# GTEC-UDC/roskfpos

Hardware: AMD Instinct MI355X
Metric: EKF predict+update steps/s at 65536 tags x 8 anchors; RMS pos err vs CPU ref (higher is better)
Workload: dtype f64 arithmetic; f64 state and covariance, f32/int32 measurements in HBM (KFPOS_STORE_MIXED)

## Files before the change

### __graft_entry__.py

```python
from __future__ import annotations

import os
import shutil
import subprocess
import sys

ROOT = os.path.dirname(os.path.abspath(__file__))
CSRC = os.path.join(ROOT, "roskfpos_amd", "csrc")
HIP_LIB = os.path.join(CSRC, "libkfpos_hip.so")
ADAPTOR_DEMO = os.path.join(CSRC, "kfpos_replay")


def _stale(target, sources):
    if not os.path.exists(target):
        return True
    mt = os.path.getmtime(target)
    return any(os.path.getmtime(s) > mt for s in sources if os.path.exists(s))


def build(force: bool = False) -> None:
    jobs = str(min(8, os.cpu_count() or 1))
    res = subprocess.run(["make", "-s", "-j", jobs, "-C", CSRC] + (["-B"] if force else []) + ["all"],
                         capture_output=True, text=True)
    if res.returncode != 0:
        sys.stderr.write(res.stdout + res.stderr)
        raise subprocess.CalledProcessError(res.returncode, res.args)
    res = subprocess.run(["make", "-s", "-C", CSRC, "check"], capture_output=True, text=True)
    if res.returncode != 0:
        sys.stderr.write(res.stdout + res.stderr)
        if os.path.exists(HIP_LIB):
            os.remove(HIP_LIB)
        raise RuntimeError("a build-time performance rule is broken (scratch inside a loop / a kernel lost its second "
                           "wavefront per SIMD): " + (res.stdout + res.stderr).strip())
    subprocess.check_call(["make", "-s", "-C", os.path.join(ROOT, "oracle")] + (["-B"] if force else []))
    import glob
    core_headers = sorted(glob.glob(os.path.join(CSRC, "kfpos_core*.h"))) + [os.path.join(CSRC, "kfpos_p48.h")]
    emu_dir = os.path.join(ROOT, "tests", "emu")
    emu_so = os.path.join(emu_dir, "libkfpos_emu.so")
    if force or _stale(emu_so, [os.path.join(emu_dir, "kfpos_emu.cpp")] + core_headers):
        subprocess.check_call(["g++", "-O2", "-std=c++17", "-fPIC", "-shared", "-Wno-unknown-pragmas",
                               "-o", emu_so, os.path.join(emu_dir, "kfpos_emu.cpp")])
    fake_dir = os.path.join(ROOT, "tests", "fake_rccl")
    fake_so = os.path.join(fake_dir, "libfake_rccl.so")
    if force or _stale(fake_so, [os.path.join(fake_dir, "fake_rccl.cpp")]):
        subprocess.check_call([shutil.which("hipcc") or "/opt/rocm/bin/hipcc", "-O2", "-std=c++17", "-shared", "-fPIC",
                               "-o", fake_so, os.path.join(fake_dir, "fake_rccl.cpp"), "-lrt"])
    if ROOT not in sys.path:
        sys.path.insert(0, ROOT)
    import roskfpos_amd
    from roskfpos_amd import capi
    capi.load()


def smoke() -> None:
    if ROOT not in sys.path:
        sys.path.insert(0, ROOT)
    sys.path.insert(0, os.path.join(ROOT, "oracle"))
    import numpy as np
    from roskfpos_amd import capi
    from roskfpos_amd.synth import Workload
    import oracle_py

    T, A, S = 256, 8, 12
    w = Workload(T, A)
    for model in (capi.MODEL_TOA, capi.MODEL_TOA_IMU):
        bank = capi.KfposBank(model, T, w.anchors, init_pos=w.init_positions())
        orc = oracle_py.OracleBank(model, T, w.anchors, init_pos=w.init_positions(), n_threads=4)
        err, cov = w.err_est(), w.accel_cov()
        for s in range(S):
            r, a, dt = w.ranges_mm(s), w.accel(s), w.dt_of(s)
            if model == capi.MODEL_TOA_IMU:
                bank.step_toa_imu(r, err, a, cov, dt)
                orc.step_imu(a, cov, 0.0)
                orc.step_toa(r, err, dt)
            else:
                bank.step_toa(r, err, dt)
                orc.step_toa(r, err, dt)
        x, _, _ = bank.get_state()
        xo, _ = orc.get_state()
        rms = float(np.sqrt(((x[:, :3] - xo[:, :3]) ** 2).sum(1).mean()))
        print(f"smoke model={model}: RMS position difference vs oracle = {rms:.3e} m")
        assert rms <= 1e-6, rms
        bank.close()


if __name__ == "__main__":
    build()
    if len(sys.argv) > 1 and sys.argv[1] == "smoke":
        smoke()
```

### roskfpos_amd/csrc/kfpos_core_imu9.h

```cpp
#ifndef KFPOS_CORE_IMU9_H
#define KFPOS_CORE_IMU9_H

namespace kfpos {

constexpr double INFO_FORM_MIN_PIVOT = 1e-7;

struct Tag9 {
    double pos[3], vel[3];
    Cov<9, true> P;
};
struct Imu {
    bool has;
    double acc[3];
    double *ci;
    int ci_stride;
    KFPOS_HD double Wi(int k) const { return ci[(6 + k) * ci_stride]; }
};

KFPOS_FN void imu_whitener(const double s[9], double *ci, int ci_stride) {
    double c00, c11, c22, i00, i11, i22;
    kf_sqrt_rsqrt(s[0], c00, i00);
    const double c10 = s[3] * i00, c20 = s[6] * i00;
    kf_sqrt_rsqrt(s[4] - c10 * c10, c11, i11);
    const double c21 = (s[7] - c20 * c10) * i11;
// ... 618 lines not shown
    Iekf9Iter it;
    KFPOS_UNROLL
    for (int k = 0; k < 6; ++k) { it.ve[k] = 0.0; it.wl[k] = 0.0; o.mrlast[k] = 0.0; }
    it.qd = 0.0;
    it.cost = 1e20;
    o.dlast[0] = o.dlast[1] = o.dlast[2] = 0.0;
    o.gain_iters = 0;
#if defined(__HIP_DEVICE_COMPILE__)
    constexpr bool PAIRS = RANGING && SC::NA == 8 && SC::CHUNK == 0 && !SC::COOP;
    const bool pairs = PAIRS && pr.pair_anchor_tab && __builtin_amdgcn_ballot_w64(true) == ~0ull;
#endif
    bool more = true;
    int stop = max_steps;
#if defined(__HIP_DEVICE_COMPILE__)
    if (pairs) stop = 8 < max_steps ? 8 : max_steps;
#endif
    for (;;) {
        while (more && o.gain_iters < stop) {
            Iekf9Parked pk;
            iekf9_fetch<false>(binv, binv_stride, imu, pk);
            const double p[3] = {xhat[0] + it.ve[0], xhat[1] + it.ve[1], xhat[2] + it.ve[2]};
            Sweep9 sw;
            iekf9_sweep<RANGING>(p, sc, pr, sw);
            more = iekf9_pass<DIAG>(xhat, pk, imu, tol, sw, it, o);
        }
#if defined(__HIP_DEVICE_COMPILE__)
        if constexpr (PAIRS) {
            if (pairs) {
                const uint64_t m = __builtin_amdgcn_ballot_w64(more && o.gain_iters < max_steps);
                if (m == 0) break;
                if (__popcll(m) <= 32) {
                    iekf9_pairs<DIAG, ACC0>(m, xhat, binv, binv_stride, sc, pr.pair_anchor_tab, imu, max_steps, tol, it, o);
                    break;
                }
                stop = stop + 4 < max_steps ? stop + 4 : max_steps;
                continue;
            }
        }
#endif
        break;
    }
    KFPOS_UNROLL
    for (int k = 0; k < 6; ++k) o.w[k] = it.wl[k];
    o.cost = it.cost;
}

KFPOS_FN void cov_update9(Cov<9, true> &P, const double mr[6], const double d[3], const Imu &imu) {
    Factor9 f;
    factor9(mr, d, imu, f);
    KFPOS_UNROLL
    for (int k = 0; k < 6; ++k) {
        double pt[9], s = 1.0;
        KFPOS_UNROLL
        for (int i = 0; i < 9; ++i) {
            double v = 0.0;
            KFPOS_UNROLL
            for (int l = 0; l < 6; ++l) {
                const bool nz = (l < 3 && k < 3 && l >= k) || (l >= 3 && k >= 3 && l <= k);
                if (nz) v += P(i, e9(l)) * L9(f, l, k);
            }
            pt[i] = v;
        }
        KFPOS_UNROLL
        for (int l = 0; l < 6; ++l) {
            const bool nz = (l < 3 && k < 3 && l >= k) || (l >= 3 && k >= 3 && l <= k);
            if (nz) s += L9(f, l, k) * pt[e9(l)];
        }
        const double is = kf_rcp(s);
        KFPOS_UNROLL
        for (int i = 0; i < 9; ++i) {
            const double pi = pt[i] * is;
            KFPOS_UNROLL
            for (int j = i; j < 9; ++j) P(i, j) -= pi * pt[j];
        }
    }
}

struct CovPark9 {
    double *a;
    int stride;
};

template <bool RANGING, class SC>
KFPOS_FN uint32_t step_imu9(Tag9 &tg, SC &sc, const Params &pr, double dt, const Imu &imu, const CovPark9 &park) {
    constexpr bool has_ranging = RANGING;
    const int n_valid = has_ranging ? count_used(sc, pr, 0) : 0;
    if (!pr.use_init_pos && (isnan(tg.pos[0]) || isnan(tg.pos[1]))) {
        if (!has_ranging) return 0;
        if (n_valid < 4) return ST_FEW_RANGES;
        double p[3] = {1.0, 1.0, 4.0}, sse, c[6];
        set_weights_ml(sc, pr, 0ull);
        const int it = ml_estimate(p, sc, pr, 0, n_valid, sse);
        if (ml_covariance_throws(sc, pr, 0, n_valid, sse)) return ST_UPDATE_SKIPPED;
        if (!ml_covariance(p, sc, pr, sse, c)) return ST_UPDATE_SKIPPED;
        tg.pos[0] = p[0]; tg.pos[1] = p[1]; tg.pos[2] = p[2];
        tg.P(0, 0) = c[0]; tg.P(0, 1) = c[1]; tg.P(1, 1) = c[3];
        return pack_status(ST_ML_INIT, 0, it, -1);
    }
    const double c = dt * dt / 2;
    double xhat[9];
    KFPOS_UNROLL
    for (int k = 0; k < 3; ++k) {
        xhat[k] = tg.pos[k] + dt * tg.vel[k] + c * 0.0;
        xhat[3 + k] = tg.vel[k] + dt * 0.0;
        xhat[6 + k] = 0.0;
    }
    predict9(tg.P, dt, pr.jolt);
    Cov<6, true> B;
    KFPOS_UNROLL
    for (int i = 0; i < 6; ++i) {
        KFPOS_UNROLL
        for (int j = i; j < 6; ++j) B(i, j) = tg.P(e9(i), e9(j));
    }
    KFPOS_UNROLL
    for (int k = 0; k < 45; ++k) park.a[k * park.stride] = tg.P.a[k];
    double *binv = park.a + 45 * park.stride;
    const bool invertible = sym6_inverse(B, binv, park.stride, INFO_FORM_MIN_PIVOT);
    Iekf9Out o;
    iekf9_weights(xhat, sc, pr, has_ranging, n_valid, o);
    if (o.flags & ST_UPDATE_SKIPPED) {
        KFPOS_UNROLL
        for (int k = 0; k < 45; ++k) tg.P.a[k] = park.a[k * park.stride];
        return ST_UPDATE_SKIPPED;
    }
    if (invertible) {
        iekf9_info<false, RANGING, true>(xhat, binv, park.stride, sc, pr, imu, 20, 1e-4, o);
        KFPOS_UNROLL
        for (int k = 0; k < 45; ++k) tg.P.a[k] = park.a[k * park.stride];
    } else {
        KFPOS_UNROLL
        for (int k = 0; k < 45; ++k) tg.P.a[k] = park.a[k * park.stride];
        iekf9<false, RANGING>(xhat, tg.P, sc, pr, imu, 20, 1e-4, o);
    }
    KFPOS_UNROLL
    for (int i = 0; i < 6; ++i) {
        double v = 0.0;
        KFPOS_UNROLL
        for (int k = 0; k < 6; ++k) v += tg.P(i, e9(k)) * o.w[k];
        if (i < 3) tg.pos[i] = xhat[i] + v;
        else tg.vel[i - 3] = xhat[i] + v;
    }
    cov_update9(tg.P, o.mrlast, o.dlast, imu);
    return pack_status(o.flags, o.gain_iters, o.ml_iters, -1);
}

KFPOS_FN void pose9(const Tag9 &tg, double t, double jolt, double pos[3], double vel[3], double cov[9]) {
    const double c = t * t / 2, t3 = (t * t * t) / 6;
    KFPOS_UNROLL
    for (int i = 0; i < 3; ++i) {
        pos[i] = tg.pos[i] + t * tg.vel[i];
        vel[i] = tg.vel[i];
        KFPOS_UNROLL
        for (int j = 0; j < 3; ++j) {
            const Cov<9, true> &P = tg.P;
            const double xpp = P(i, j) + t * P(3 + i, j) + c * P(6 + i, j);
            const double xpv = P(i, 3 + j) + t * P(3 + i, 3 + j) + c * P(6 + i, 3 + j);
            const double xpa = P(i, 6 + j) + t * P(3 + i, 6 + j) + c * P(6 + i, 6 + j);
            cov[3 * i + j] = xpp + t * xpv + c * xpa + (i == j ? jolt * t3 * t3 : 0.0);
        }
    }
}

}
#endif
```

### roskfpos_amd/csrc/kfpos_hip.hip

```cpp
#include <algorithm>
#include <cmath>
#include <cstdio>
#include <cstdlib>
#include <cstring>
#include <new>
#include <string>
#include <type_traits>
#include <vector>

#include "kfpos_kernels.h"

std::string &kfpos_error_text() {
    thread_local std::string text;
    return text;
}

namespace {

#define g_err (kfpos_error_text())

#define HIPCHK(expr)                                                                              \
    do {                                                                                          \
        hipError_t e_ = (expr);                                                                   \
        if (e_ != hipSuccess) {                                                                   \
            g_err = std::string(#expr) + ": " + hipGetErrorString(e_);                            \
            return KFPOS_ERR_HIP;                                                                 \
        }                                                                                         \
    } while (0)

}


namespace {

size_t lds_bytes(const kfpos_handle *h) { return (size_t)3 * h->cfg.max_anchors * WAVE * sizeof(double); }
size_t park_bytes() { return (size_t)36 * WAVE * sizeof(double); }
size_t park9_bytes() { return (size_t)78 * WAVE * sizeof(double) + 24 * sizeof(double); }

void fill_args(const kfpos_handle *h, KArgs &a) {
    std::memcpy(a.anchors, h->anchors, sizeof(a.anchors));
    a.T = h->cfg.n_tags;
    a.A = h->have_anchors ? h->A : 0;
    a.accel_noise = h->cfg.accel_noise;
    a.jolt = h->cfg.jolt;
    a.cost_threshold = h->cfg.cost_threshold;
    a.ignore_worst = h->cfg.ignore_worst;
    a.top_n = h->cfg.top_n;
    a.ml_variant = h->cfg.model == KFPOS_MODEL_ML ? h->cfg.ml_variant : 0;
    a.pair9 = h->pair9 ? 1 : 0;
    a.use_init_pos = h->cfg.use_init_pos;
    a.use_fixed_height = h->planar.use_fixed_height;
    a.imu_fixed_cov_acc = h->planar.imu_use_fixed_cov_acc;
    a.imu_fixed_cov_w = h->planar.imu_use_fixed_cov_ang_vel_z;
    a.px4_height = h->planar.px4_height;
    a.px4_arm_p1 = h->planar.px4_arm_p1;
    a.px4_arm_p2 = h->planar.px4_arm_p2;
    a.px4_cov_vel = h->planar.px4_cov_velocity;
    a.px4_cov_gyro_z = h->planar.px4_cov_gyro_z;
    a.imu_cov_acc = h->planar.imu_cov_acc;
    a.imu_cov_w = h->planar.imu_cov_ang_vel_z;
    a.mag_offset = h->planar.mag_angle_offset;
    a.mag_cov = h->planar.mag_cov;
    a.platch = h->d_latch;
    a.sensor = nullptr;
    a.pos = h->d_pos;
    a.vel = h->d_vel;
    a.P = h->d_P;
    a.flags = h->d_flags;
    a.imu_acc = h->d_imu_acc;
    a.imu_cov = h->d_imu_cov;
    a.ranges = nullptr;
    a.err = nullptr;
    a.dt = nullptr;
    a.dt_shared = 0.0;
    a.accel = nullptr;
    a.cov = nullptr;
    a.mode = MODE_TOA;
    a.latch = 1;
    a.status = nullptr;
    a.n_steps = 1;
    a.stride_ranges = a.stride_err = a.stride_accel = a.stride_cov = 0;
    a.traj = nullptr;
}


bool toa6_two_waves(const kfpos_handle *h) {
    return h->two_waves && h->cfg.model == KFPOS_MODEL_TOA && !h->full && !h->force_generic && !h->coop &&
           h->cfg.max_anchors == 8 && h->cfg.ignore_worst == 0 && h->cfg.top_n == 0;
}
int static_anchors(const kfpos_handle *h) {
    if (h->cfg.max_anchors == 8) return 8;
    if (h->cfg.max_anchors == 16 && h->cfg.model == KFPOS_MODEL_TOA) return -16;
    return 0;
}

step_kernel_t step_kernel(const kfpos_handle *h, bool sensor_call = false, bool imu_only = false) {
    const int st = h->cfg.storage, as = (h->force_generic || sensor_call) ? 0 : static_anchors(h);
    if (h->cfg.model == KFPOS_MODEL_PLANAR) return kfpos_k::planar_kernel(st, h->planar_sensors || sensor_call, as);
    if (h->cfg.model == KFPOS_MODEL_ML) return kfpos_k::ml_kernel(st, as);
    if (h->coop) return kfpos_k::toa6_coop_kernel(st);
    if (h->cfg.model == KFPOS_MODEL_TOA) {
        const int heur = h->cfg.ignore_worst != 0 ? 2 : (h->cfg.top_n != 0 ? 1 : 0);
        if (h->full) return kfpos_k::toa6_full_kernel(st, as, heur);
        return kfpos_k::toa6_sym_kernel(st, as, heur, toa6_two_waves(h));
    }
    return kfpos_k::imu9_kernel(st, as, !imu_only);
}

int launch_step(kfpos_handle *h, const KArgs &a, hipStream_t s) {
    if (h->coop) {
        const int groups = (a.T + COOP_TAGS_PER_WAVE - 1) / COOP_TAGS_PER_WAVE;
        hipLaunchKernelGGL(step_kernel(h), dim3(groups), dim3(WAVE), 0, s, a);
        HIPCHK(hipGetLastError());
        h->stepped = true;
        return KFPOS_OK;
    }
    const int blocks = (a.T + WAVE - 1) / WAVE;
    const bool generic = h->force_generic || static_anchors(h) <= 0 || (h->cfg.model == KFPOS_MODEL_TOA && h->full) ||
                         (h->cfg.model == KFPOS_MODEL_PLANAR && h->planar_sensors) || toa6_two_waves(h);
    const bool planar_sensor = h->cfg.model == KFPOS_MODEL_PLANAR && a.mode != 0;
    size_t lds = (a.mode == MODE_IMU_ONLY || planar_sensor || !generic) ? 0 : lds_bytes(h);
    if (lds && h->cfg.model == KFPOS_MODEL_TOA && !h->force_generic && static_anchors(h) != 0 && h->msz == 4)
        lds = lds * 5 / 6;
    if (h->cfg.model == KFPOS_MODEL_PLANAR && (h->planar_sensors || planar_sensor)) lds += park_bytes();
    if (h->cfg.model == KFPOS_MODEL_TOA && h->full) lds += park_bytes();
    if (toa6_two_waves(h)) lds += (size_t)(h->msz == 4 ? 19 : 15) * WAVE * sizeof(double);
    if (h->cfg.model == KFPOS_MODEL_TOA_IMU) lds += park9_bytes();
    hipLaunchKernelGGL(step_kernel(h, planar_sensor, a.mode == MODE_IMU_ONLY && h->cfg.model == KFPOS_MODEL_TOA_IMU), dim3(blocks), dim3(WAVE), lds, s, a);
    HIPCHK(hipGetLastError());
    h->stepped = true;
    return KFPOS_OK;
}
// ... 116 lines not shown

inline int pidx(const kfpos_handle *h, int i, int j) {
    if (h->full) return i * h->n + j;
    const int N = h->n;
    if (i > j) { const int tt = i; i = j; j = tt; }
    return i * N - i * (i - 1) / 2 + (j - i);
}

}

extern "C" {

const char *kfpos_last_error(void) { return g_err.c_str(); }
const char *kfpos_strerror(int code) {
    switch (code) {
    case KFPOS_OK: return "ok";
    case KFPOS_ERR_ARG: return "invalid argument";
    case KFPOS_ERR_HIP: return "HIP runtime error";
    case KFPOS_ERR_NO_DEVICE: return "no usable GPU";
    case KFPOS_ERR_MODEL: return "call not defined for this model";
    case KFPOS_ERR_STATE: return "call out of sequence";
    case KFPOS_ERR_COMM: return "RCCL error";
    default: return "unknown error";
    }
}
int kfpos_version(void) { return KFPOS_VERSION; }

int kfpos_create(const kfpos_config *cfg, kfpos_handle **out) {
    if (!cfg || !out) return KFPOS_ERR_ARG;
    *out = nullptr;
    g_err.clear();
    auto bad = [](const char *why) {
        g_err = why;
        return KFPOS_ERR_ARG;
    };
    if (cfg->model != KFPOS_MODEL_TOA && cfg->model != KFPOS_MODEL_TOA_IMU && cfg->model != KFPOS_MODEL_ML &&
        cfg->model != KFPOS_MODEL_PLANAR)
        return bad("kfpos_config.model is not one of KFPOS_MODEL_*");
    if (cfg->storage != KFPOS_STORE_F64 && cfg->storage != KFPOS_STORE_F32 && cfg->storage != KFPOS_STORE_MIXED &&
        cfg->storage != KFPOS_STORE_P48)
        return bad("kfpos_config.storage is not one of KFPOS_STORE_*");
    if (cfg->n_tags < 1) return bad("kfpos_config.n_tags must be >= 1");
    if (cfg->max_anchors < 1 || cfg->max_anchors > KFPOS_MAX_ANCHORS)
        return bad("kfpos_config.max_anchors must be 1..64 (MAX_NUM_ANCS, Posgenerator.h:74)");
    if (cfg->top_n < 0) return bad("kfpos_config.top_n must be >= 0");
    if (cfg->ml_variant != KFPOS_ML_NORMAL && cfg->ml_variant != KFPOS_ML_IGNORE_N && cfg->ml_variant != KFPOS_ML_BEST)
        return bad("kfpos_config.ml_variant is not one of KFPOS_ML_*");
    if (cfg->ml_variant != KFPOS_ML_NORMAL && cfg->model != KFPOS_MODEL_ML)
        return bad("kfpos_config.ml_variant belongs to KFPOS_MODEL_ML (MLLocation's variants, MLLocation.h:5-7)");
    if ((cfg->model == KFPOS_MODEL_TOA_IMU && (cfg->top_n || cfg->ignore_worst)) ||
        (cfg->model == KFPOS_MODEL_ML && cfg->ignore_worst) ||
        (cfg->model == KFPOS_MODEL_PLANAR && (cfg->top_n || cfg->ignore_worst)))
        return bad("ignore_worst exists for the 6-state filter only, top_n for the 6-state filter and the ML estimator");
    int ndev = 0;
    if (hipGetDeviceCount(&ndev) != hipSuccess || ndev <= 0 || cfg->device < 0 || cfg->device >= ndev) {
        g_err = "no HIP device";
        return KFPOS_ERR_NO_DEVICE;
    }
    DevScope dev_(cfg->device);
    kfpos_handle *h = new (std::nothrow) kfpos_handle();
    if (!h) return KFPOS_ERR_ARG;
    h->cfg = *cfg;
    h->n = cfg->model == KFPOS_MODEL_TOA_IMU ? 9 : (cfg->model == KFPOS_MODEL_ML ? 3 : (cfg->model == KFPOS_MODEL_PLANAR ? 8 : 6));
    h->full = (cfg->model == KFPOS_MODEL_TOA && !cfg->use_init_pos) ? 1 : 0;
    h->psz = h->full ? h->n * h->n : h->n * (h->n + 1) / 2;
    h->rsz = cfg->storage == KFPOS_STORE_F32 ? 4 : (cfg->storage == KFPOS_STORE_P48 ? 6 : 8);
    h->msz = cfg->storage == KFPOS_STORE_F64 ? 8 : 4;
    h->A = 0;
    h->have_anchors = false;
    h->stepped = false;
    {
        const char *g = getenv("KFPOS_GENERIC_KERNEL");
        h->force_generic = g && g[0] == '1';
        if (h->full && cfg->ignore_worst && cfg->storage == KFPOS_STORE_P48) h->force_generic = true;
        {
            hipDeviceProp_t prop;
            const char *ow = getenv("KFPOS_ONE_WAVE_BUILD");
            h->two_waves = false;
            if (!(ow && ow[0] == '1') && hipGetDeviceProperties(&prop, cfg->device) == hipSuccess)
                h->two_waves = ((size_t)cfg->n_tags + WAVE - 1) / WAVE > (size_t)prop.multiProcessorCount * 4;
        }
        const char *np = getenv("KFPOS_PAIR9");
        h->pair9 = np && np[0] == '1';
        const char *nc = getenv("KFPOS_NO_COOP");
        h->coop = !(nc && nc[0] == '1') && !h->force_generic && cfg->model == KFPOS_MODEL_TOA && cfg->use_init_pos &&
                  !cfg->ignore_worst && !cfg->top_n && cfg->max_anchors <= COOP_LANES && cfg->n_tags <= 8192;
        const char *c = getenv("KFPOS_TRACE_CHUNK_STEPS");
        int n = c ? atoi(c) : KFPOS_TRACE_CHUNK;
        h->trace_chunk = n < 1 ? 1 : (n > KFPOS_TRACE_CHUNK ? KFPOS_TRACE_CHUNK : n);
    }
    std::memset(h->anchors, 0, sizeof(h->anchors));
    const size_t T = cfg->n_tags, A = cfg->max_anchors, r = h->rsz, m = h->msz;
#define ALLOC(ptr, bytes)                                                     \
    do {                                                                      \
        hipError_t e_ = hipMalloc((void **)&(ptr), (bytes));                  \
        if (e_ != hipSuccess) {                                               \
            g_err = std::string("hipMalloc: ") + hipGetErrorString(e_);       \
            kfpos_destroy(h);                                                 \
            return KFPOS_ERR_HIP;                                             \
        }                                                                     \
        (void)hipMemset((ptr), 0, (bytes));                                   \
    } while (0)
    ALLOC(h->d_pos, 3 * T * sizeof(double));
    ALLOC(h->d_P, h->psz * T * r);
    ALLOC(h->d_flags, T * sizeof(uint32_t));
    if (h->n == 3) ALLOC(h->d_vel, 3 * T * sizeof(double));
    if (h->n == 8) {
        ALLOC(h->d_vel, 4 * T * sizeof(double));
        ALLOC(h->d_latch, LATCH_ROWS * T * sizeof(double));
        ALLOC(h->d_sensor, 24 * T * sizeof(double));
    }
    if (h->n == 9) {
        ALLOC(h->d_vel, 3 * T * sizeof(double));
        ALLOC(h->d_imu_acc, 3 * T * m);
        ALLOC(h->d_imu_cov, 6 * T * m);
        ALLOC(h->d_accel, 3 * T * m);
        ALLOC(h->d_cov, 9 * T * m);
    }
    ALLOC(h->d_ranges, A * T * sizeof(int32_t));
    ALLOC(h->d_err, A * T * m);
    ALLOC(h->d_dt, T * sizeof(double));
    ALLOC(h->d_out, 15 * T * sizeof(double));
    ALLOC(h->d_status, T * sizeof(uint32_t));
#undef ALLOC
    if (hipEventCreate(&h->ev0) != hipSuccess || hipEventCreate(&h->ev1) != hipSuccess) {
        g_err = "hipEventCreate failed";
        kfpos_destroy(h);
        return KFPOS_ERR_HIP;
    }
    if (T * A <= small_bank_limit()) {
        size_t off = 0;
        auto region = [&](size_t bytes) { const size_t o = off; off += (bytes + 255) & ~(size_t)255; return o; };
        h->sm_ranges = region(A * T * sizeof(int32_t));
        h->sm_err = region(A * T * m);
        h->sm_accel = region(3 * T * m);
        h->sm_cov = region(9 * T * m);
        h->sm_dt = region(T * sizeof(double));
        h->sm_sensor = region(24 * T * sizeof(double));
        h->sm_status = region(T * sizeof(uint32_t));
        h->sm_out = region((size_t)(15 + h->n + h->n * h->n) * T * sizeof(double));
        void *hp = nullptr, *dp = nullptr;
        if (hipHostMalloc(&hp, off, hipHostMallocMapped) != hipSuccess || hipHostGetDevicePointer(&dp, hp, 0) != hipSuccess) {
            g_err = "hipHostMalloc(mapped block of a small bank) failed";
            if (hp) (void)hipHostFree(hp);
            kfpos_destroy(h);
            return KFPOS_ERR_HIP;
        }
        std::memset(hp, 0, off);
        h->sm_h = (unsigned char *)hp;
        h->sm_bytes = off;
        h->sm_d = (unsigned char *)dp;
    }
    const bool parks = cfg->model == KFPOS_MODEL_PLANAR || (cfg->model == KFPOS_MODEL_TOA && h->full);
    if (cfg->model == KFPOS_MODEL_TOA_IMU && lds_bytes(h) + park9_bytes() > 64 * 1024) {
        hipError_t e_ = hipFuncSetAttribute((const void *)step_kernel(h), hipFuncAttributeMaxDynamicSharedMemorySize,
                                            (int)(lds_bytes(h) + park9_bytes()));
        if (e_ != hipSuccess) {
            g_err = std::string("hipFuncSetAttribute: ") + hipGetErrorString(e_);
            kfpos_destroy(h);
            return KFPOS_ERR_HIP;
        }
    } else if (lds_bytes(h) + (parks ? park_bytes() : 0) > 64 * 1024) {
        hipError_t e_ = hipFuncSetAttribute((const void *)step_kernel(h), hipFuncAttributeMaxDynamicSharedMemorySize,
                                            (int)(lds_bytes(h) + (h->full ? park_bytes() : 0)));
        if (e_ == hipSuccess && cfg->model == KFPOS_MODEL_PLANAR) {
            h->planar_sensors = true;
// ... 1447 lines not shown
```

### roskfpos_amd/csrc/kfpos_internal.h

```cpp
#ifndef KFPOS_INTERNAL_H
#define KFPOS_INTERNAL_H

#include <hip/hip_runtime.h>

#include <string>
#include <vector>

#include "../../include/kfpos.h"

#define KFPOS_TRACE_CHUNK 128
#define KFPOS_N_SLOTS 3

__attribute__((visibility("hidden"))) std::string &kfpos_error_text();

struct KfposDevScope {
    int prev = -1;
    bool switched = false;
    explicit KfposDevScope(int dev) {
        if (hipGetDevice(&prev) == hipSuccess && prev != dev) switched = hipSetDevice(dev) == hipSuccess;
    }
    ~KfposDevScope() {
        if (switched) (void)hipSetDevice(prev);
    }
    KfposDevScope(const KfposDevScope &) = delete;
    KfposDevScope &operator=(const KfposDevScope &) = delete;
};

struct kfpos_handle {
    kfpos_config cfg;
    int n;
    int full;
    int psz;
    int rsz;
    int msz;
    int A;
    bool have_anchors, stepped;
    int trace_chunk;
    bool force_generic;
    bool two_waves;
    bool pair9;
    bool coop;
    double anchors[KFPOS_MAX_ANCHORS * 3];
    double *d_pos = nullptr;
    double *d_vel = nullptr;
    void *d_P = nullptr, *d_imu_acc = nullptr, *d_imu_cov = nullptr;
    uint32_t *d_flags = nullptr;
    int32_t *d_ranges = nullptr;
    void *d_err = nullptr, *d_accel = nullptr, *d_cov = nullptr;
    double *d_dt = nullptr, *d_out = nullptr;
    uint32_t *d_status = nullptr;
    hipEvent_t ev0 = nullptr, ev1 = nullptr;
    kfpos_planar_config planar = {};
    bool planar_sensors = false;
    double *d_latch = nullptr;
    double *d_sensor = nullptr;
    unsigned char *d_stage = nullptr;
    size_t stage_cap = 0, stage_used = 0;
    unsigned char *sm_h = nullptr, *sm_d = nullptr;
    size_t sm_ranges = 0, sm_err = 0, sm_accel = 0, sm_cov = 0, sm_dt = 0, sm_sensor = 0, sm_status = 0, sm_out = 0;
    size_t sm_bytes = 0;
    struct Slot {
        unsigned char *host = nullptr;
        unsigned char *dev = nullptr;
        hipEvent_t copied = nullptr, copied2 = nullptr, computed = nullptr, done = nullptr;
        hipEvent_t err_reader = nullptr, cov_reader = nullptr;
        bool busy = false;
        int32_t *rows = nullptr;
    } slot[KFPOS_N_SLOTS];
    size_t so_ranges = 0, so_err = 0, so_accel = 0, so_cov = 0, so_dt = 0, so_status = 0, so_pos = 0, so_bytes = 0;
    hipStream_t s_copy = nullptr, s_copy2 = nullptr, s_comp = nullptr, s_back = nullptr;
    size_t split_bytes = 0;
    int err_slot = -1, cov_slot = -1;
    unsigned char *d_work = nullptr;
    size_t work_cap = 0;
    std::vector<uint32_t> row_stamp;
    uint32_t stamp = 0;
};

#endif
```

### roskfpos_amd/csrc/kfpos_k_imu9.hip

```cpp
#include "kfpos_kernels.h"

namespace {

template <typename MREAL>
struct RawImu {
    MREAL acc[3];
};
template <typename MREAL>
__device__ inline void fetch_imu(const KArgs &a, size_t t, int s, RawImu<MREAL> &raw) {
    const MREAL *ap = (const MREAL *)a.accel + (size_t)s * a.stride_accel;
#pragma unroll
    for (int k = 0; k < 3; ++k) raw.acc[k] = (ap + (size_t)k * a.T)[(uint32_t)t];
}
template <typename MREAL>
__device__ inline void fetch_imu_cov(const KArgs &a, size_t t, int s, MREAL raw[9]) {
    const MREAL *cp = (const MREAL *)a.cov + (size_t)s * a.stride_cov;
#pragma unroll
    for (int k = 0; k < 9; ++k) raw[k] = (cp + (size_t)k * a.T)[(uint32_t)t];
}
template <typename MREAL>
__device__ inline void latch_imu_cov(const KArgs &a, size_t T, uint32_t t32, const double cv[9]) {
    strow<MREAL>(a.imu_cov, 0, T, t32, cv[0]);
    strow<MREAL>(a.imu_cov, 1, T, t32, cv[3]);
    strow<MREAL>(a.imu_cov, 2, T, t32, cv[4]);
    strow<MREAL>(a.imu_cov, 3, T, t32, cv[6]);
    strow<MREAL>(a.imu_cov, 4, T, t32, cv[7]);
    strow<MREAL>(a.imu_cov, 5, T, t32, cv[8]);
}

template <typename REAL, typename MREAL, int AS, bool RANGING = true>
__global__ __launch_bounds__(WAVE) void k_step_imu9(const KArgs a) {
    extern __shared__ double lds[];
    const int lane = threadIdx.x;
    const size_t t = (size_t)blockIdx.x * WAVE + lane;
    if (t >= (size_t)a.T) return;
    const size_t T = a.T;
    const uint32_t t32 = (uint32_t)t;
    Params pr = make_params(a);
    constexpr bool has_ranging = RANGING;
    constexpr bool AHEAD = sizeof(MREAL) == 4 && !std::is_same<REAL, float>::value;
    const bool fresh_imu = a.mode != MODE_TOA;
    constexpr int NA = AS > 0 ? AS : 1;
    if (a.n_steps == 1 && a.dt && a.dt[t32] < 0.0) {
        skipped_lane(a, t, true);
        return;
    }

    uint32_t fl = a.flags[t32];
    RawEpoch<MREAL, NA> raw;
    RawImu<MREAL> rawi;
    if constexpr (AS > 0) {
        if (has_ranging) fetch_epoch<MREAL, AS>(a, t, 0, raw);
    }
    Tag9 tg;
#pragma unroll
    for (int k = 0; k < 3; ++k) {
        tg.pos[k] = (a.pos + k * T)[t32];
        tg.vel[k] = (a.vel + k * T)[t32];
    }
    const CovPark9 park{lds + ((AS == 0 && has_ranging) ? 3 * (size_t)a.A * WAVE : 0) + lane, WAVE};
    Imu imu;
    imu.has = false;
    imu.ci = park.a + 66 * WAVE;
    imu.ci_stride = WAVE;
    if constexpr (AS == 8 && RANGING) {
        if (a.pair9) {
            double *tab = lds + 78 * WAVE;
#pragma unroll
            for (int k = 0; k < 24; ++k) tab[k] = a.anchors[k];
            pr.pair_anchor_tab = tab;
        }
    }
    double cv[9] = {1, 0, 0, 0, 1, 0, 0, 0, 1};
    MREAL rawc[9];
    if (fresh_imu) {
        fetch_imu<MREAL>(a, t, 0, rawi);
        fetch_imu_cov<MREAL>(a, t, 0, rawc);
    } else if (fl & FL_HAS_IMU) {
        imu.has = true;
#pragma unroll
        for (int k = 0; k < 3; ++k) imu.acc[k] = ldrow<MREAL>(a.imu_acc, k, T, t32);
        cv[0] = ldrow<MREAL>(a.imu_cov, 0, T, t32);
        cv[3] = ldrow<MREAL>(a.imu_cov, 1, T, t32);
        cv[4] = ldrow<MREAL>(a.imu_cov, 2, T, t32);
        cv[6] = ldrow<MREAL>(a.imu_cov, 3, T, t32);
        cv[7] = ldrow<MREAL>(a.imu_cov, 4, T, t32);
        cv[8] = ldrow<MREAL>(a.imu_cov, 5, T, t32);
    }
#pragma unroll
    for (int k = 0; k < 45; ++k) tg.P.a[k] = ldcov<REAL>(a.P, k, 45, T, t32);
    if (fresh_imu) {
        imu.has = true;
#pragma unroll
        for (int k = 0; k < 9; ++k) cv[k] = (double)rawc[k];
        if (a.latch) latch_imu_cov<MREAL>(a, T, t32, cv);
    }
    if (imu.has) imu_whitener(cv, imu.ci, imu.ci_stride);


    uint32_t s = 0;
    for (int e = 0; e < a.n_steps; ++e) {
        const double dt = epoch_dt(a, t, e);
        if (fresh_imu) {
#pragma unroll
            for (int k = 0; k < 3; ++k) imu.acc[k] = (double)rawi.acc[k];
            if (e + 1 < a.n_steps) {
                if constexpr (AHEAD) fetch_imu<MREAL>(a, opaque_lane(t), opaque_uniform(e + 1), rawi);
            }
        }
        if constexpr (AS > 0) {
            RegScratch<AS> sc;
            if (has_ranging) {
                unpack_epoch<MREAL, AS>(raw, sc);
                if (e + 1 < a.n_steps) {
                    if constexpr (AHEAD) fetch_epoch<MREAL, AS>(a, opaque_lane(t), opaque_uniform(e + 1), raw);
                }
            } else {
#pragma unroll
                for (int k = 0; k < AS; ++k) sc.r[k] = sc.e[k] = sc.w[k] = 0.0;
            }
            s = step_imu9<RANGING>(tg, sc, pr, dt, imu, park);
            if constexpr (!AHEAD) {
                if (e + 1 < a.n_steps) {
                    if (fresh_imu) fetch_imu<MREAL>(a, opaque_lane(t), opaque_uniform(e + 1), rawi);
                    if (has_ranging) fetch_epoch<MREAL, AS>(a, opaque_lane(t), opaque_uniform(e + 1), raw);
                }
            }
        } else {
            Scratch sc{nullptr, nullptr, nullptr, WAVE};
            if (has_ranging) sc = stage_epoch_lds<MREAL>(a, lds, lane, t, opaque_uniform(e));
            s = step_imu9<RANGING>(tg, sc, pr, dt, imu, park);
            if constexpr (!AHEAD) {
                if (e + 1 < a.n_steps && fresh_imu) fetch_imu<MREAL>(a, opaque_lane(t), opaque_uniform(e + 1), rawi);
            }
        }
        if (a.traj) {
#pragma unroll
            for (int k = 0; k < 3; ++k) (a.traj + ((size_t)opaque_uniform(e) * 3 + k) * T)[t32] = tg.pos[k];
        }
        if constexpr (cov_is_rounded<REAL>()) {
            if (e + 1 < a.n_steps) {
#pragma unroll
                for (int k = 0; k < 45; ++k) tg.P.a[k] = round_cov<REAL>(tg.P.a[k]);
            }
        }
    }

    if (fresh_imu && a.latch) {
#pragma unroll
        for (int k = 0; k < 3; ++k) strow<MREAL>(a.imu_acc, k, T, t32, imu.acc[k]);
        fl |= FL_HAS_IMU;
    }
    bool fin = true;
#pragma unroll
    for (int k = 0; k < 3; ++k) {
        (a.pos + k * T)[t32] = tg.pos[k];
        (a.vel + k * T)[t32] = tg.vel[k];
        fin &= isfinite(tg.pos[k]) & isfinite(tg.vel[k]);
    }
#pragma unroll
    for (int k = 0; k < 45; ++k) {
        stcov<REAL>(a.P, k, 45, T, t32, tg.P.a[k]);
        fin &= isfinite(tg.P.a[k]);
    }
    const bool waiting = !a.use_init_pos && isnan(tg.pos[0]);
    if (!fin && !waiting) s |= ST_NONFINITE;
    a.flags[t32] = fl | FL_STARTED;
    if (a.status) a.status[t32] = s;
}

}

template <typename REAL, typename MREAL>
static kfpos_k::step_kernel_t imu9_of(int as, bool ranging) {
    if (!ranging) return k_step_imu9<REAL, MREAL, 0, false>;
    if (as == 8) return k_step_imu9<REAL, MREAL, 8>;
    return k_step_imu9<REAL, MREAL, 0>;
}
kfpos_k::step_kernel_t kfpos_k::imu9_kernel(int st, int as, bool ranging) {
    return KFPOS_BY_STORAGE(st, imu9_of, as, ranging);
}
```

### roskfpos_amd/csrc/kfpos_kernels.h

```cpp
#ifndef KFPOS_KERNELS_H
#define KFPOS_KERNELS_H

#include <hip/hip_runtime.h>

#include <cmath>
#include <cstdint>
#include <type_traits>

#define KFPOS_HD __host__ __device__
#include "kfpos_core.h"
#include "kfpos_internal.h"
#include "kfpos_p48.h"

namespace kfpos_k {

struct KArgs {
    double anchors[KFPOS_MAX_ANCHORS * 3];
    int T, A;
    double accel_noise, jolt, cost_threshold;
    int ignore_worst, top_n, use_init_pos, ml_variant;
    int pair9;
    int use_fixed_height, imu_fixed_cov_acc, imu_fixed_cov_w;
    double px4_height, px4_arm_p1, px4_arm_p2, px4_cov_vel, px4_cov_gyro_z;
    double imu_cov_acc, imu_cov_w, mag_offset, mag_cov;
    double *platch;
    const double *sensor;
    double *pos;
    double *vel;
    void *P;
    uint32_t *flags;
    void *imu_acc;
    void *imu_cov;
    const int32_t *ranges;
    const void *err;
    const double *dt;
    double dt_shared;
    const void *accel;
    const void *cov;
    int mode, latch;
    uint32_t *status;
    int n_steps;
    long long stride_ranges, stride_err, stride_accel, stride_cov;
    double *traj;
    double dt_steps[KFPOS_TRACE_CHUNK];
};


struct PoseArgs {
    int T, model, full;
    double accel_noise, jolt, dt_ahead;
    const double *dt_each;
    const double *pos_in;
    const double *vel_in;
    const void *P;
    const uint32_t *flags;
    double *pos, *cov, *vel;
    double *full_x, *full_P;
    uint32_t *status;
};

typedef void (*step_kernel_t)(const KArgs);

step_kernel_t toa6_sym_kernel(int st, int as, int heur, bool two_waves);
step_kernel_t toa6_full_kernel(int st, int as, int heur);
step_kernel_t toa6_coop_kernel(int st);
step_kernel_t imu9_kernel(int st, int as, bool ranging);
step_kernel_t ml_kernel(int st, int as);
step_kernel_t planar_kernel(int st, bool sensors, int as);
void launch_get_pose(int model, bool full, int st, int blocks, hipStream_t s, const PoseArgs &a);
void launch_rows_to_cols(size_t esz, hipStream_t s, const void *src, void *dst, int T, int C);
void launch_cols_to_rows(hipStream_t s, const double *src, double *dst, int T, int C);

struct TagComp {
    uint8_t kind, buf, row, aux;
};
enum : int { TC_NONE = 0, TC_F64 = 1, TC_COV = 2, TC_REAL = 3 };
enum : int { TB_POS = 0, TB_VEL, TB_P, TB_IMU_ACC, TB_IMU_COV, TB_LATCH, TB_N };
enum : int { TAGS_GATHER = 0, TAGS_SCATTER = 1, TAGS_RESET = 2, TAGS_WORK_IN = 3, TAGS_WORK_OUT = 4 };
constexpr int TAG_SECTIONS = 4;
constexpr int TAG_COMPS = 9 + 81 + 15 + 1;
struct TagArgs {
    int T, n, psz;
    int w[TAG_SECTIONS];
    int cbase[TAG_SECTIONS];
    int n_comp;
    void *buf[TB_N];
    uint32_t *flags;
    const int32_t *rows;
    double *val;
    uint32_t *fl;
    const double *init;
    double cst[5];
    void *wbuf[TB_N];
    uint32_t *wflags;
    TagComp comp[TAG_COMPS];
};
void launch_tags(int op, int st, hipStream_t s, const TagArgs &a);

constexpr int COOP_LANES = 8;
constexpr int COOP_TAGS_PER_WAVE = 64 / COOP_LANES;
constexpr int PLANAR_HAS_SHIFT = 4;
constexpr int LATCH_ROWS = 15;

}
// ... 189 lines not shown
```

Before: 1.946 billion.

## Use diagonal IMU covariance fast path and restructure 9-state epoch loop prefetching

Splits the 9-state IMU step into a state update and a covariance update. It adds a wave-uniform check (via ballot) that lets the IEKF take a diagonal-whitener specialisation when every lane's IMU covariance has zero off-diagonal terms. It also hoists the per-epoch dt load one step ahead, issues the IMU prefetch alongside the ranging epoch fetch, and inserts an explicit waitcnt before the loop. The diagonal path is on by default, can be turned off with KFPOS_IMU9_DIAG=0, and adds template instantiations that raise code size and may change register pressure.

```diff
diff --git a/__graft_entry__.py b/__graft_entry__.py
--- a/__graft_entry__.py
+++ b/__graft_entry__.py
@@ -31,7 +31,7 @@
         if os.path.exists(HIP_LIB):
             os.remove(HIP_LIB)
         raise RuntimeError("a build-time performance rule is broken (scratch inside a loop / a kernel lost its second "
-                           "wavefront per SIMD): " + (res.stdout + res.stderr).strip())
+                           "wavefront per SIMD / the 9-state epoch loop waits for a memory operation just issued): " + (res.stdout + res.stderr).strip())
     subprocess.check_call(["make", "-s", "-C", os.path.join(ROOT, "oracle")] + (["-B"] if force else []))
     import glob
     core_headers = sorted(glob.glob(os.path.join(CSRC, "kfpos_core*.h"))) + [os.path.join(CSRC, "kfpos_p48.h")]
diff --git a/roskfpos_amd/csrc/kfpos_core_imu9.h b/roskfpos_amd/csrc/kfpos_core_imu9.h
--- a/roskfpos_amd/csrc/kfpos_core_imu9.h
+++ b/roskfpos_amd/csrc/kfpos_core_imu9.h
@@ -724,20 +724,25 @@
 };
 
 template <bool RANGING, class SC>
-KFPOS_FN uint32_t step_imu9(Tag9 &tg, SC &sc, const Params &pr, double dt, const Imu &imu, const CovPark9 &park) {
+KFPOS_FN bool step_imu9_state(Tag9 &tg, SC &sc, const Params &pr, double dt, const Imu &imu, const CovPark9 &park,
+                              bool diag, Iekf9Out &o, uint32_t &status) {
     constexpr bool has_ranging = RANGING;
     const int n_valid = has_ranging ? count_used(sc, pr, 0) : 0;
     if (!pr.use_init_pos && (isnan(tg.pos[0]) || isnan(tg.pos[1]))) {
-        if (!has_ranging) return 0;
-        if (n_valid < 4) return ST_FEW_RANGES;
+        status = 0;
+        if (!has_ranging) return false;
+        status = ST_FEW_RANGES;
+        if (n_valid < 4) return false;
         double p[3] = {1.0, 1.0, 4.0}, sse, c[6];
         set_weights_ml(sc, pr, 0ull);
         const int it = ml_estimate(p, sc, pr, 0, n_valid, sse);
-        if (ml_covariance_throws(sc, pr, 0, n_valid, sse)) return ST_UPDATE_SKIPPED;
-        if (!ml_covariance(p, sc, pr, sse, c)) return ST_UPDATE_SKIPPED;
+        status = ST_UPDATE_SKIPPED;
+        if (ml_covariance_throws(sc, pr, 0, n_valid, sse)) return false;
+        if (!ml_covariance(p, sc, pr, sse, c)) return false;
         tg.pos[0] = p[0]; tg.pos[1] = p[1]; tg.pos[2] = p[2];
         tg.P(0, 0) = c[0]; tg.P(0, 1) = c[1]; tg.P(1, 1) = c[3];
-        return pack_status(ST_ML_INIT, 0, it, -1);
+        status = pack_status(ST_ML_INIT, 0, it, -1);
+        return false;
     }
     const double c = dt * dt / 2;
     double xhat[9];
@@ -758,21 +763,23 @@
     for (int k = 0; k < 45; ++k) park.a[k * park.stride] = tg.P.a[k];
     double *binv = park.a + 45 * park.stride;
     const bool invertible = sym6_inverse(B, binv, park.stride, INFO_FORM_MIN_PIVOT);
-    Iekf9Out o;
     iekf9_weights(xhat, sc, pr, has_ranging, n_valid, o);
     if (o.flags & ST_UPDATE_SKIPPED) {
         KFPOS_UNROLL
         for (int k = 0; k < 45; ++k) tg.P.a[k] = park.a[k * park.stride];
-        return ST_UPDATE_SKIPPED;
+        status = ST_UPDATE_SKIPPED;
+        return false;
     }
     if (invertible) {
-        iekf9_info<false, RANGING, true>(xhat, binv, park.stride, sc, pr, imu, 20, 1e-4, o);
+        if (diag) iekf9_info<true, RANGING, true>(xhat, binv, park.stride, sc, pr, imu, 20, 1e-4, o);
+        else iekf9_info<false, RANGING, true>(xhat, binv, park.stride, sc, pr, imu, 20, 1e-4, o);
         KFPOS_UNROLL
         for (int k = 0; k < 45; ++k) tg.P.a[k] = park.a[k * park.stride];
     } else {
         KFPOS_UNROLL
         for (int k = 0; k < 45; ++k) tg.P.a[k] = park.a[k * park.stride];
-        iekf9<false, RANGING>(xhat, tg.P, sc, pr, imu, 20, 1e-4, o);
+        if (diag) iekf9<true, RANGING>(xhat, tg.P, sc, pr, imu, 20, 1e-4, o);
+        else iekf9<false, RANGING>(xhat, tg.P, sc, pr, imu, 20, 1e-4, o);
     }
     KFPOS_UNROLL
     for (int i = 0; i < 6; ++i) {
@@ -782,8 +789,19 @@
         if (i < 3) tg.pos[i] = xhat[i] + v;
         else tg.vel[i - 3] = xhat[i] + v;
     }
+    status = 0;
+    return true;
+}
+KFPOS_FN uint32_t step_imu9_cov(Tag9 &tg, const Iekf9Out &o, const Imu &imu) {
     cov_update9(tg.P, o.mrlast, o.dlast, imu);
     return pack_status(o.flags, o.gain_iters, o.ml_iters, -1);
+}
+template <bool RANGING, class SC>
+KFPOS_FN uint32_t step_imu9(Tag9 &tg, SC &sc, const Params &pr, double dt, const Imu &imu, const CovPark9 &park) {
+    Iekf9Out o;
+    uint32_t status;
+    if (!step_imu9_state<RANGING>(tg, sc, pr, dt, imu, park, false, o, status)) return status;
+    return step_imu9_cov(tg, o, imu);
 }
 
 KFPOS_FN void pose9(const Tag9 &tg, double t, double jolt, double pos[3], double vel[3], double cov[9]) {
diff --git a/roskfpos_amd/csrc/kfpos_hip.hip b/roskfpos_amd/csrc/kfpos_hip.hip
--- a/roskfpos_amd/csrc/kfpos_hip.hip
+++ b/roskfpos_amd/csrc/kfpos_hip.hip
@@ -48,6 +48,7 @@
     a.top_n = h->cfg.top_n;
     a.ml_variant = h->cfg.model == KFPOS_MODEL_ML ? h->cfg.ml_variant : 0;
     a.pair9 = h->pair9 ? 1 : 0;
+    a.imu9_diag = h->imu9_diag ? 1 : 0;
     a.use_init_pos = h->cfg.use_init_pos;
     a.use_fixed_height = h->planar.use_fixed_height;
     a.imu_fixed_cov_acc = h->planar.imu_use_fixed_cov_acc;
@@ -330,6 +331,8 @@
         }
         const char *np = getenv("KFPOS_PAIR9");
         h->pair9 = np && np[0] == '1';
+        const char *nd = getenv("KFPOS_IMU9_DIAG");
+        h->imu9_diag = !(nd && nd[0] == '0');
         const char *nc = getenv("KFPOS_NO_COOP");
         h->coop = !(nc && nc[0] == '1') && !h->force_generic && cfg->model == KFPOS_MODEL_TOA && cfg->use_init_pos &&
                   !cfg->ignore_worst && !cfg->top_n && cfg->max_anchors <= COOP_LANES && cfg->n_tags <= 8192;
diff --git a/roskfpos_amd/csrc/kfpos_internal.h b/roskfpos_amd/csrc/kfpos_internal.h
--- a/roskfpos_amd/csrc/kfpos_internal.h
+++ b/roskfpos_amd/csrc/kfpos_internal.h
@@ -39,6 +39,7 @@
     bool force_generic;
     bool two_waves;
     bool pair9;
+    bool imu9_diag;
     bool coop;
     double anchors[KFPOS_MAX_ANCHORS * 3];
     double *d_pos = nullptr;
diff --git a/roskfpos_amd/csrc/kfpos_k_imu9.hip b/roskfpos_amd/csrc/kfpos_k_imu9.hip
--- a/roskfpos_amd/csrc/kfpos_k_imu9.hip
+++ b/roskfpos_amd/csrc/kfpos_k_imu9.hip
@@ -41,9 +41,13 @@
     constexpr bool AHEAD = sizeof(MREAL) == 4 && !std::is_same<REAL, float>::value;
     const bool fresh_imu = a.mode != MODE_TOA;
     constexpr int NA = AS > 0 ? AS : 1;
-    if (a.n_steps == 1 && a.dt && a.dt[t32] < 0.0) {
-        skipped_lane(a, t, true);
-        return;
+    double dt_tag = a.dt_shared;
+    if (a.n_steps == 1 && a.dt) {
+        dt_tag = a.dt[t32];
+        if (dt_tag < 0.0) {
+            skipped_lane(a, t, true);
+            return;
+        }
     }
 
     uint32_t fl = a.flags[t32];
@@ -96,30 +100,53 @@
         if (a.latch) latch_imu_cov<MREAL>(a, T, t32, cv);
     }
     if (imu.has) imu_whitener(cv, imu.ci, imu.ci_stride);
-
-
+    bool diag = false;
+    if (a.imu9_diag) {
+        const bool mine = !imu.has || (imu.Wi(1) == 0.0 && imu.Wi(2) == 0.0 && imu.Wi(4) == 0.0);
+        diag = __builtin_amdgcn_ballot_w64(mine) == __builtin_amdgcn_ballot_w64(true);
+    }
+
+    const bool multi = a.n_steps > 1;
+    double dt_next = multi ? a.dt_steps[0] : dt_tag;
+    constexpr bool IMU_WITH_EPOCH = AHEAD && AS > 0 && RANGING;
+
+    __builtin_amdgcn_s_waitcnt(0x0F70);
     uint32_t s = 0;
     for (int e = 0; e < a.n_steps; ++e) {
-        const double dt = epoch_dt(a, t, e);
+        const double dt = dt_next;
+        if (multi && e + 1 < a.n_steps) dt_next = a.dt_steps[opaque_uniform(e + 1)];
         if (fresh_imu) {
 #pragma unroll
             for (int k = 0; k < 3; ++k) imu.acc[k] = (double)rawi.acc[k];
-            if (e + 1 < a.n_steps) {
-                if constexpr (AHEAD) fetch_imu<MREAL>(a, opaque_lane(t), opaque_uniform(e + 1), rawi);
-            }
-        }
+            if constexpr (AHEAD && !IMU_WITH_EPOCH) {
+                if (e + 1 < a.n_steps) fetch_imu<MREAL>(a, opaque_lane(t), opaque_uniform(e + 1), rawi);
+            }
+        }
+        Iekf9Out o;
+        auto finish = [&](bool update) {
+            if (a.traj) {
+#pragma unroll
+                for (int k = 0; k < 3; ++k) (a.traj + ((size_t)opaque_uniform(e) * 3 + k) * T)[t32] = tg.pos[k];
+            }
+            if (update) s = step_imu9_cov(tg, o, imu);
+        };
         if constexpr (AS > 0) {
             RegScratch<AS> sc;
             if (has_ranging) {
                 unpack_epoch<MREAL, AS>(raw, sc);
                 if (e + 1 < a.n_steps) {
-                    if constexpr (AHEAD) fetch_epoch<MREAL, AS>(a, opaque_lane(t), opaque_uniform(e + 1), raw);
+                    if constexpr (AHEAD) {
+                        fetch_epoch<MREAL, AS>(a, opaque_lane(t), opaque_uniform(e + 1), raw);
+                        if constexpr (IMU_WITH_EPOCH) {
+                            if (fresh_imu) fetch_imu<MREAL>(a, opaque_lane(t), opaque_uniform(e + 1), rawi);
+                        }
+                    }
                 }
             } else {
 #pragma unroll
                 for (int k = 0; k < AS; ++k) sc.r[k] = sc.e[k] = sc.w[k] = 0.0;
             }
-            s = step_imu9<RANGING>(tg, sc, pr, dt, imu, park);
+            finish(step_imu9_state<RANGING>(tg, sc, pr, dt, imu, park, diag, o, s));
             if constexpr (!AHEAD) {
                 if (e + 1 < a.n_steps) {
                     if (fresh_imu) fetch_imu<MREAL>(a, opaque_lane(t), opaque_uniform(e + 1), rawi);
@@ -129,14 +156,10 @@
         } else {
             Scratch sc{nullptr, nullptr, nullptr, WAVE};
             if (has_ranging) sc = stage_epoch_lds<MREAL>(a, lds, lane, t, opaque_uniform(e));
-            s = step_imu9<RANGING>(tg, sc, pr, dt, imu, park);
+            finish(step_imu9_state<RANGING>(tg, sc, pr, dt, imu, park, diag, o, s));
             if constexpr (!AHEAD) {
                 if (e + 1 < a.n_steps && fresh_imu) fetch_imu<MREAL>(a, opaque_lane(t), opaque_uniform(e + 1), rawi);
             }
-        }
-        if (a.traj) {
-#pragma unroll
-            for (int k = 0; k < 3; ++k) (a.traj + ((size_t)opaque_uniform(e) * 3 + k) * T)[t32] = tg.pos[k];
         }
         if constexpr (cov_is_rounded<REAL>()) {
             if (e + 1 < a.n_steps) {
diff --git a/roskfpos_amd/csrc/kfpos_kernels.h b/roskfpos_amd/csrc/kfpos_kernels.h
--- a/roskfpos_amd/csrc/kfpos_kernels.h
+++ b/roskfpos_amd/csrc/kfpos_kernels.h
@@ -20,6 +20,7 @@
     double accel_noise, jolt, cost_threshold;
     int ignore_worst, top_n, use_init_pos, ml_variant;
     int pair9;
+    int imu9_diag;
     int use_fixed_height, imu_fixed_cov_acc, imu_fixed_cov_w;
     double px4_height, px4_arm_p1, px4_arm_p2, px4_cov_vel, px4_cov_gyro_z;
     double imu_cov_acc, imu_cov_w, mag_offset, mag_cov;
```

Result: faster. 2.024 billion (median of 6 runs) (+4.1%).
